# eth-cscs/DLA-Future

Measured on AMD Instinct MI355X. Metric: cholesky_fp64_gflops, higher is better.
Workload: dtype fp64; 1 GPU; model=fp64 Cholesky (POTRF), n=32768, nb=512, parallelism=grid1x1, global_batch=1, seq_len=32768

## Files before the change

csrc/factor.hip:

```cpp
#include <algorithm>

#include "kernels.h"
#include "potrf_plan.h"

namespace {

template <typename S, int BSZ>
__launch_bounds__(256) __global__ void trtri_block_lds_k(const S* L, S* T,
                                                         int n, int ldl,
                                                         int ldt,
                                                         int unit_diag) {
  using TR = ScalarTraits<S>;
  __shared__ S Ts[BSZ][BSZ + 1];
  const int tid = threadIdx.x;
  const int j = tid;
  if (j < n) {
    for (int i = 0; i < j; ++i) Ts[i][j] = TR::zero();
    const S djj = unit_diag ? TR::from_real(1) : TR::recip(L[(int64_t)j * ldl + j]);
    Ts[j][j] = djj;
    for (int i = j + 1; i < n; ++i) {
      S acc = TR::zero();
      const S* Lrow = L + (int64_t)i * ldl;
      for (int p = j; p < i; ++p) acc += Lrow[p] * Ts[p][j];
      const S dii = unit_diag ? TR::from_real(1) : TR::recip(L[(int64_t)i * ldl + i]);
      Ts[i][j] = -(dii * acc);
    }
  }
  __syncthreads();
  for (int e = tid; e < BSZ * BSZ; e += 256) {
    const int i = e / BSZ, j2 = e % BSZ;
    if (i < n && j2 < n) T[(int64_t)i * ldt + j2] = Ts[i][j2];
  }
}

constexpr int kB = dlaf::kPotrfBsz;
constexpr int kImgLd = kB + 1;
static_assert(kB == 64, "the core below is written for 64 x 64 blocks");

template <typename S>
using Img = S (*)[kImgLd];

template <typename S>
__device__ __forceinline__ S read_lane(S v, int src) {
  constexpr int NW = sizeof(S) / 4;
  int w[NW];
  __builtin_memcpy(w, &v, sizeof(S));
#pragma unroll
  for (int q = 0; q < NW; ++q) w[q] = __builtin_amdgcn_readlane(w[q], src);
  __builtin_memcpy(&v, w, sizeof(S));
  return v;
}

__device__ __forceinline__ double pivot_rcp(double a) {
  double x = __builtin_amdgcn_rcp(a);
  double e = fma(-a, x, 1.0);
  x = fma(x, e, x);
  e = fma(-a, x, 1.0);
  return fma(x, e, x);
}
__device__ __forceinline__ float pivot_rcp(float a) { return 1.0f / a; }

template <typename S>
__device__ inline void factor16_wave(Img<S> L,
                                     typename ScalarTraits<S>::real_t* rdiag,
                                     int c0, int lane) {
  using TR = ScalarTraits<S>;
  using RT = typename TR::real_t;
  const int i = lane & 15;
  S u[16];
#pragma unroll
  for (int j = 0; j < 16; ++j) u[j] = L[c0 + i][c0 + j];
#pragma unroll
  for (int p = 0; p < 15; ++p) {
    const RT s = pivot_rcp(TR::real(read_lane(u[p], p)));
    const S w = u[p] * s;
#pragma unroll
    for (int j = p + 1; j < 16; ++j)
      u[j] -= w * TR::conj(read_lane(u[p], j));
  }
  RT dv = RT(0);
#pragma unroll
  for (int j = 0; j < 16; ++j)
    if (i == j) dv = TR::real(u[j]);
  const RT sc = RT(1) / sqrt(dv);
#pragma unroll
  for (int j = 0; j < 16; ++j) u[j] = u[j] * read_lane(sc, j);
  if (lane < 16) {
#pragma unroll
    for (int j = 0; j < 16; ++j)
      if (j <= i) L[c0 + i][c0 + j] = u[j];
    rdiag[c0 + i] = sc;
  }
}

template <typename S>
__device__ inline void invert16_wave(Img<S> L, Img<S> T, int c0, int lane) {
  using TR = ScalarTraits<S>;
  const int i = lane & 15;
  S l[16], t[16];
#pragma unroll
  for (int j = 0; j < 16; ++j) l[j] = L[c0 + i][c0 + j];
  S dv = TR::from_real(1);
#pragma unroll
  for (int j = 0; j < 16; ++j)
    if (i == j) dv = l[j];
  const S rd = TR::recip(dv);
#pragma unroll
  for (int c = 0; c < 16; ++c) t[c] = (c == i) ? rd : TR::zero();
#pragma unroll
  for (int p = 0; p < 15; ++p) {
    const S f = rd * l[p];
#pragma unroll
    for (int c = 0; c <= p; ++c) {
      const S tp = read_lane(t[c], p);
      if (i > p) t[c] -= f * tp;
    }
  }
  if (lane < 16) {
#pragma unroll
    for (int c = 0; c < 16; ++c)
      T[c0 + i][c0 + c] = (c <= i) ? t[c] : TR::zero();
  }
}

template <typename S>
__device__ void factor_invert_core(Img<S> L, Img<S> T, S (*Sc)[33],
                                   typename ScalarTraits<S>::real_t* rdiag,
                                   int tid, int do_factor) {
  using TR = ScalarTraits<S>;
  for (int e = tid; e < kB * kImgLd; e += 256) (&T[0][0])[e] = TR::zero();
  if (do_factor) {
    for (int cb = 0; cb < 4; ++cb) {
      const int c0 = cb * 16;
      if (tid < 64) factor16_wave<S>(L, rdiag, c0, tid);
      __syncthreads();
      if (cb == 3) break;
      {
        const int r = c0 + 16 + tid;
        if (r < kB) {
          S a[16];
#pragma unroll
          for (int p = 0; p < 16; ++p) a[p] = L[r][c0 + p];
#pragma unroll
          for (int j = 0; j < 16; ++j) {
            a[j] = a[j] * rdiag[c0 + j];
#pragma unroll
            for (int q = j + 1; q < 16; ++q)
              a[q] -= a[j] * TR::conj(L[c0 + q][c0 + j]);
          }
#pragma unroll
          for (int p = 0; p < 16; ++p) L[r][c0 + p] = a[p];
        }
        __syncthreads();
      }
      {
        const int t0 = c0 + 16, m = 3 - cb;
        const int ti = tid >> 4, tj = tid & 15;
        for (int bi = 0; bi < m; ++bi) {
          S xi[16];
#pragma unroll
          for (int p = 0; p < 16; ++p) xi[p] = L[t0 + 16 * bi + ti][c0 + p];
          for (int bj = 0; bj <= bi; ++bj) {
            if (bj == bi && tj > ti) continue;
            const int rj = t0 + 16 * bj + tj;
            S acc = TR::zero();
#pragma unroll
            for (int p = 0; p < 16; ++p) acc += xi[p] * TR::conj(L[rj][c0 + p]);
            L[t0 + 16 * bi + ti][rj] -= acc;
          }
        }
        __syncthreads();
      }
    }
  } else {
    __syncthreads();
  }
  invert16_wave<S>(L, T, (tid >> 6) * 16, tid & 63);
  __syncthreads();
  for (int dist = 1; dist < 4; ++dist) {
    const int nblk = 4 - dist;
    for (int e = tid; e < nblk * 256; e += 256) {
      const int b = e >> 8, r = (e & 255) >> 4, c = e & 15;
      const int I = (b + dist) * 16, J = b * 16;
      S acc = TR::zero();
      for (int p = J; p < I; ++p) acc += L[I + r][p] * T[p][J + c];
      Sc[(b >> 1) * 16 + r][(b & 1) * 16 + c] = acc;
    }
    __syncthreads();
    for (int e = tid; e < nblk * 256; e += 256) {
      const int b = e >> 8, r = (e & 255) >> 4, c = e & 15;
      const int I = (b + dist) * 16, J = b * 16;
      S acc = TR::zero();
      for (int p = 0; p <= r; ++p)
        acc += T[I + r][I + p] * Sc[(b >> 1) * 16 + p][(b & 1) * 16 + c];
      T[I + r][J + c] = -acc;
    }
    __syncthreads();
  }
}

template <typename S>
__device__ inline void store_factor_and_inverse(Img<S> L, Img<S> T, S* A,
                                                int n, int ld, S* Tout,
                                                int tid, int store_factor) {
  for (int e = tid; e < kB * kB; e += 256) {
    const int i = e >> 6, j = e & 63;
    if (store_factor && i < n && j <= i) A[(int64_t)i * ld + j] = L[i][j];
    Tout[e] = T[i][j];
  }
}

template <typename S>
__launch_bounds__(256) __global__ void potrf_invert_block_k(S* A, int n,
                                                            int ld, S* Tout,
                                                            int do_factor) {
  using TR = ScalarTraits<S>;
  __shared__ S Li[kB][kImgLd];
  __shared__ S Ti[kB][kImgLd];
  __shared__ S Sc[32][33];
  __shared__ typename TR::real_t Rd[kB];
  const int tid = threadIdx.x;
  for (int e = tid; e < kB * kB; e += 256) {
    const int i = e >> 6, j = e & 63;
    Li[i][j] = (i < n && j <= i) ? A[(int64_t)i * ld + j]
                                 : (i == j ? TR::from_real(1) : TR::zero());
  }
  __syncthreads();
  factor_invert_core<S>(Li, Ti, Sc, Rd, tid, do_factor);
  store_factor_and_inverse<S>(Li, Ti, A, n, ld, Tout, tid, do_factor);
}

template <typename S>
__launch_bounds__(256) __global__ void potrf_step_k(S* A, int n, int ld,
                                                    S* dinv, S* side, int d,
                                                    int nbk) {
  using TR = ScalarTraits<S>;
  namespace plan = dlaf::potrf_plan;
  __shared__ S P0[kB][kImgLd];
  __shared__ S P1[kB][kImgLd];
  __shared__ S Sc[32][33];
  __shared__ typename TR::real_t Rd[kB];
  const int tid = threadIdx.x;
  int I, J;
  plan::block_of((int)blockIdx.x, nbk, d, &I, &J);
  const int c = d - 1;
  const int r0 = I * kB, s0 = J * kB, q0 = c * kB;

  for (int R = d - 1; R < nbk; ++R) {
    if (!plan::copies_row(I, J, nbk, d, R)) continue;
    const S* src = side + plan::side_offset((d - 2) & 1, R, nbk, kB);
    for (int e = tid; e < kB * kB; e += 256) {
      const int i = e >> 6, j = e & 63;
      if (R * kB + i < n)
        A[(int64_t)(R * kB + i) * ld + (q0 - kB) + j] = src[e];
    }
  }

  const S* Dc = dinv + (int64_t)c * kB * kB;
  for (int e = tid; e < kB * kB; e += 256) {
    const int i = e >> 6, j = e & 63;
    P0[i][j] = (r0 + i < n) ? A[(int64_t)(r0 + i) * ld + q0 + j] : TR::zero();
    P1[i][j] = Dc[e];
  }
  __syncthreads();

  const int ty = tid >> 4, tx = tid & 15;
  auto panel_product = [&](S (&x)[4][4]) {
#pragma unroll
    for (int a = 0; a < 4; ++a)
#pragma unroll
      for (int b = 0; b < 4; ++b) x[a][b] = TR::zero();
#pragma unroll
    for (int pb = 0; pb < 4; ++pb) {
      for (int pp = 0; pp < 16; ++pp) {
        const int p = pb * 16 + pp;
        S av[4];
#pragma unroll
        for (int a = 0; a < 4; ++a) av[a] = P0[ty + 16 * a][p];
#pragma unroll
        for (int b = pb; b < 4; ++b) {
          const S dv = TR::conj(P1[tx + 16 * b][p]);
#pragma unroll
          for (int a = 0; a < 4; ++a) x[a][b] += av[a] * dv;
        }
      }
    }
  };

  S xi[4][4], xj[4][4];
  panel_product(xi);
  __syncthreads();
  if (I != J) {
    for (int e = tid; e < kB * kB; e += 256) {
      const int i = e >> 6, j = e & 63;
      P0[i][j] = (s0 + i < n) ? A[(int64_t)(s0 + i) * ld + q0 + j] : TR::zero();
    }
    __syncthreads();
    panel_product(xj);
    __syncthreads();
  }
#pragma unroll
  for (int a = 0; a < 4; ++a)
#pragma unroll
    for (int b = 0; b < 4; ++b) {
      P0[ty + 16 * a][tx + 16 * b] = xi[a][b];
      P1[ty + 16 * a][tx + 16 * b] = (I != J) ? xj[a][b] : xi[a][b];
    }
  if (plan::writes_side(I, J, nbk, d)) {
    S* dst = side + plan::side_offset(c & 1, I, nbk, kB);
#pragma unroll
    for (int a = 0; a < 4; ++a)
#pragma unroll
      for (int b = 0; b < 4; ++b)
        dst[(ty + 16 * a) * kB + tx + 16 * b] = xi[a][b];
  } else if (plan::writes_panel_in_place(I, J, nbk, d)) {
#pragma unroll
    for (int a = 0; a < 4; ++a)
#pragma unroll
      for (int b = 0; b < 4; ++b)
        if (r0 + ty + 16 * a < n)
          A[(int64_t)(r0 + ty + 16 * a) * ld + q0 + tx + 16 * b] = xi[a][b];
  }
  __syncthreads();

  S cv[4][4];
#pragma unroll
  for (int a = 0; a < 4; ++a)
#pragma unroll
    for (int b = 0; b < 4; ++b) {
      const int gr = r0 + ty + 16 * a, gc = s0 + tx + 16 * b;
      const bool live = gr < n && gc < n && (I != J || gc <= gr);
      cv[a][b] = live ? A[(int64_t)gr * ld + gc] : TR::zero();
    }
  for (int q = 0; q < kB; ++q) {
    S av[4], bv[4];
#pragma unroll
    for (int a = 0; a < 4; ++a) av[a] = P0[ty + 16 * a][q];
#pragma unroll
    for (int b = 0; b < 4; ++b) bv[b] = TR::conj(P1[tx + 16 * b][q]);
#pragma unroll
    for (int a = 0; a < 4; ++a)
#pragma unroll
      for (int b = 0; b < 4; ++b) cv[a][b] -= av[a] * bv[b];
  }

  if (!plan::factors(I, J, d)) {
#pragma unroll
    for (int a = 0; a < 4; ++a)
#pragma unroll
      for (int b = 0; b < 4; ++b) {
        const int gr = r0 + ty + 16 * a, gc = s0 + tx + 16 * b;
        if (gr < n && gc < n && (I != J || gc <= gr))
          A[(int64_t)gr * ld + gc] = cv[a][b];
      }
    return;
  }

  __syncthreads();
  const int nl = min(kB, n - r0);
#pragma unroll
  for (int a = 0; a < 4; ++a)
#pragma unroll
    for (int b = 0; b < 4; ++b) {
      const int i = ty + 16 * a, j = tx + 16 * b;
      P0[i][j] = (i < nl && j <= i) ? cv[a][b]
                                    : (i == j ? TR::from_real(1) : TR::zero());
    }
  __syncthreads();
  factor_invert_core<S>(P0, P1, Sc, Rd, tid, 1);
  store_factor_and_inverse<S>(P0, P1, A + (int64_t)r0 * ld + r0, nl, ld,
                              dinv + (int64_t)d * kB * kB, tid, 1);
}

template <typename S>
__global__ void trtri_lower_k(const S* L, S* T, int n, int ldl, int ldt,
                              int unit_diag) {
  using TR = ScalarTraits<S>;
  const int j = blockIdx.x * blockDim.x + threadIdx.x;
  if (j >= n) return;
  for (int i = 0; i < j; ++i) T[(int64_t)i * ldt + j] = TR::zero();
  const S djj = unit_diag ? TR::from_real(1) : TR::recip(L[(int64_t)j * ldl + j]);
  T[(int64_t)j * ldt + j] = djj;
  for (int i = j + 1; i < n; ++i) {
    S acc = TR::zero();
    for (int p = j; p < i; ++p)
      acc += L[(int64_t)i * ldl + p] * T[(int64_t)p * ldt + j];
    const S dii = unit_diag ? TR::from_real(1) : TR::recip(L[(int64_t)i * ldl + i]);
    T[(int64_t)i * ldt + j] = -(dii * acc);
  }
}

}

template <typename S>
void dlaf::potrf_invert_block(S* A, int n, int ld, S* Tout, int do_factor,
                              hipStream_t stream) {
  potrf_invert_block_k<S><<<1, 256, 0, stream>>>(A, n, ld, Tout, do_factor);
}

template <typename S>
void dlaf::potrf_tile_fused(S* A, int n, int ld, S* dinv, S* side,
                            hipStream_t stream) {
  namespace plan = dlaf::potrf_plan;
  if (n <= 0) return;
  const int nbk = plan::nblocks(n, kPotrfBsz);
  potrf_invert_block_k<S>
      <<<1, 256, 0, stream>>>(A, std::min(n, kPotrfBsz), ld, dinv, 1);
  for (int d = 1; d < nbk; ++d)
    potrf_step_k<S>
        <<<plan::grid(nbk, d), 256, 0, stream>>>(A, n, ld, dinv, side, d, nbk);
}

template <typename S>
void dlaf::trtri_lower(const S* L, S* T, int n, int ldl, int ldt,
                       int unit_diag, hipStream_t stream) {
  constexpr int BSZ = sizeof(S) == 16 ? 64 : 128;
  if (n <= BSZ)
    trtri_block_lds_k<S, BSZ>
        <<<1, 256, 0, stream>>>(L, T, n, ldl, ldt, unit_diag);
  else
    trtri_lower_k<S>
        <<<(n + 255) / 256, 256, 0, stream>>>(L, T, n, ldl, ldt, unit_diag);
}

#define INSTANTIATE(S)                                                       \
  template void dlaf::potrf_invert_block(S*, int, int, S*, int, hipStream_t); \
  template void dlaf::potrf_tile_fused(S*, int, int, S*, S*, hipStream_t);    \
  template void dlaf::trtri_lower(const S*, S*, int, int, int, int, hipStream_t);
INSTANTIATE(double)
INSTANTIATE(float)
INSTANTIATE(cplx<double>)
INSTANTIATE(cplx<float>)
#undef INSTANTIATE
```

Baseline: 55190 GFlop/s.

## Use MFMA instructions in potrf step kernel and factor-invert core for real types

```diff
diff --git a/csrc/factor.hip b/csrc/factor.hip
--- a/csrc/factor.hip
+++ b/csrc/factor.hip
@@ -1,6 +1,7 @@
 #include <algorithm>
-
-#include "kernels.h"
+#include <type_traits>
+
+#include "gemm_common.h"
 #include "potrf_plan.h"
 
 namespace {
@@ -41,6 +42,9 @@
 using Img = S (*)[kImgLd];
 
 template <typename S>
+constexpr bool kOnMfma = std::is_same_v<S, double> || std::is_same_v<S, float>;
+
+template <typename S>
 __device__ __forceinline__ S read_lane(S v, int src) {
   constexpr int NW = sizeof(S) / 4;
   int w[NW];
@@ -153,7 +157,28 @@
         }
         __syncthreads();
       }
-      {
+      if constexpr (kOnMfma<S>) {
+        using MF = Mfma<S>;
+        const int t0 = c0 + 16, m = 3 - cb;
+        const int w = tid >> 6, li = tid & 15, lk = (tid & 63) >> 4;
+        for (int e = w; e < m * (m + 1) / 2; e += 4) {
+          const int bi = e >= 3 ? 2 : (e >= 1 ? 1 : 0);
+          const int bj = e - bi * (bi + 1) / 2;
+          const int ri = t0 + 16 * bi, rj = t0 + 16 * bj;
+          typename MF::acc_t c;
+#pragma unroll
+          for (int r = 0; r < 4; ++r) c[r] = L[ri + MF::acc_row(lk, r)][rj + li];
+#pragma unroll
+          for (int k = 0; k < 16; k += 4)
+            c = MF::mma(-L[ri + li][c0 + k + lk], L[rj + li][c0 + k + lk], c);
+#pragma unroll
+          for (int r = 0; r < 4; ++r) {
+            const int row = MF::acc_row(lk, r);
+            if (bj < bi || li <= row) L[ri + row][rj + li] = c[r];
+          }
+        }
+        __syncthreads();
+      } else {
         const int t0 = c0 + 16, m = 3 - cb;
         const int ti = tid >> 4, tj = tid & 15;
         for (int bi = 0; bi < m; ++bi) {
@@ -179,12 +204,26 @@
   __syncthreads();
   for (int dist = 1; dist < 4; ++dist) {
     const int nblk = 4 - dist;
-    for (int e = tid; e < nblk * 256; e += 256) {
-      const int b = e >> 8, r = (e & 255) >> 4, c = e & 15;
-      const int I = (b + dist) * 16, J = b * 16;
-      S acc = TR::zero();
-      for (int p = J; p < I; ++p) acc += L[I + r][p] * T[p][J + c];
-      Sc[(b >> 1) * 16 + r][(b & 1) * 16 + c] = acc;
+    if constexpr (kOnMfma<S>) {
+      using MF = Mfma<S>;
+      const int b = tid >> 6, li = tid & 15, lk = (tid & 63) >> 4;
+      if (b < nblk) {
+        const int I = (b + dist) * 16, J = b * 16;
+        typename MF::acc_t c = {0, 0, 0, 0};
+        for (int p = J; p < I; p += 4)
+          c = MF::mma(L[I + li][p + lk], T[p + lk][J + li], c);
+#pragma unroll
+        for (int r = 0; r < 4; ++r)
+          Sc[(b >> 1) * 16 + MF::acc_row(lk, r)][(b & 1) * 16 + li] = c[r];
+      }
+    } else {
+      for (int e = tid; e < nblk * 256; e += 256) {
+        const int b = e >> 8, r = (e & 255) >> 4, c = e & 15;
+        const int I = (b + dist) * 16, J = b * 16;
+        S acc = TR::zero();
+        for (int p = J; p < I; ++p) acc += L[I + r][p] * T[p][J + c];
+        Sc[(b >> 1) * 16 + r][(b & 1) * 16 + c] = acc;
+      }
     }
     __syncthreads();
     for (int e = tid; e < nblk * 256; e += 256) {
@@ -231,6 +270,236 @@
 }
 
 template <typename S>
+__device__ void step_block_vector(S* A, int n, int ld, S* dinv, S* side, int d,
+                                  int nbk, int I, int J, Img<S> P0, Img<S> P1,
+                                  S (*Sc)[33],
+                                  typename ScalarTraits<S>::real_t* Rd,
+                                  int tid) {
+  using TR = ScalarTraits<S>;
+  namespace plan = dlaf::potrf_plan;
+  const int c = d - 1;
+  const int r0 = I * kB, s0 = J * kB, q0 = c * kB;
+  const int ty = tid >> 4, tx = tid & 15;
+  auto panel_product = [&](S (&x)[4][4]) {
+#pragma unroll
+    for (int a = 0; a < 4; ++a)
+#pragma unroll
+      for (int b = 0; b < 4; ++b) x[a][b] = TR::zero();
+#pragma unroll
+    for (int pb = 0; pb < 4; ++pb) {
+      for (int pp = 0; pp < 16; ++pp) {
+        const int p = pb * 16 + pp;
+        S av[4];
+#pragma unroll
+        for (int a = 0; a < 4; ++a) av[a] = P0[ty + 16 * a][p];
+#pragma unroll
+        for (int b = pb; b < 4; ++b) {
+          const S dv = TR::conj(P1[tx + 16 * b][p]);
+#pragma unroll
+          for (int a = 0; a < 4; ++a) x[a][b] += av[a] * dv;
+        }
+      }
+    }
+  };
+
+  S xi[4][4], xj[4][4];
+  panel_product(xi);
+  __syncthreads();
+  if (I != J) {
+    for (int e = tid; e < kB * kB; e += 256) {
+      const int i = e >> 6, j = e & 63;
+      P0[i][j] = (s0 + i < n) ? A[(int64_t)(s0 + i) * ld + q0 + j] : TR::zero();
+    }
+    __syncthreads();
+    panel_product(xj);
+    __syncthreads();
+  }
+#pragma unroll
+  for (int a = 0; a < 4; ++a)
+#pragma unroll
+    for (int b = 0; b < 4; ++b) {
+      P0[ty + 16 * a][tx + 16 * b] = xi[a][b];
+      P1[ty + 16 * a][tx + 16 * b] = (I != J) ? xj[a][b] : xi[a][b];
+    }
+  if (plan::writes_side(I, J, nbk, d)) {
+    S* dst = side + plan::side_offset(c & 1, I, nbk, kB);
+#pragma unroll
+    for (int a = 0; a < 4; ++a)
+#pragma unroll
+      for (int b = 0; b < 4; ++b)
+        dst[(ty + 16 * a) * kB + tx + 16 * b] = xi[a][b];
+  } else if (plan::writes_panel_in_place(I, J, nbk, d)) {
+#pragma unroll
+    for (int a = 0; a < 4; ++a)
+#pragma unroll
+      for (int b = 0; b < 4; ++b)
+        if (r0 + ty + 16 * a < n)
+          A[(int64_t)(r0 + ty + 16 * a) * ld + q0 + tx + 16 * b] = xi[a][b];
+  }
+  __syncthreads();
+
+  S cv[4][4];
+#pragma unroll
+  for (int a = 0; a < 4; ++a)
+#pragma unroll
+    for (int b = 0; b < 4; ++b) {
+      const int gr = r0 + ty + 16 * a, gc = s0 + tx + 16 * b;
+      const bool live = gr < n && gc < n && (I != J || gc <= gr);
+      cv[a][b] = live ? A[(int64_t)gr * ld + gc] : TR::zero();
+    }
+  for (int q = 0; q < kB; ++q) {
+    S av[4], bv[4];
+#pragma unroll
+    for (int a = 0; a < 4; ++a) av[a] = P0[ty + 16 * a][q];
+#pragma unroll
+    for (int b = 0; b < 4; ++b) bv[b] = TR::conj(P1[tx + 16 * b][q]);
+#pragma unroll
+    for (int a = 0; a < 4; ++a)
+#pragma unroll
+      for (int b = 0; b < 4; ++b) cv[a][b] -= av[a] * bv[b];
+  }
+
+  if (!plan::factors(I, J, d)) {
+#pragma unroll
+    for (int a = 0; a < 4; ++a)
+#pragma unroll
+      for (int b = 0; b < 4; ++b) {
+        const int gr = r0 + ty + 16 * a, gc = s0 + tx + 16 * b;
+        if (gr < n && gc < n && (I != J || gc <= gr))
+          A[(int64_t)gr * ld + gc] = cv[a][b];
+      }
+    return;
+  }
+
+  __syncthreads();
+  const int nl = min(kB, n - r0);
+#pragma unroll
+  for (int a = 0; a < 4; ++a)
+#pragma unroll
+    for (int b = 0; b < 4; ++b) {
+      const int i = ty + 16 * a, j = tx + 16 * b;
+      P0[i][j] = (i < nl && j <= i) ? cv[a][b]
+                                    : (i == j ? TR::from_real(1) : TR::zero());
+    }
+  __syncthreads();
+  factor_invert_core<S>(P0, P1, Sc, Rd, tid, 1);
+  store_factor_and_inverse<S>(P0, P1, A + (int64_t)r0 * ld + r0, nl, ld,
+                              dinv + (int64_t)d * kB * kB, tid, 1);
+}
+
+template <typename S>
+__device__ void step_block_mfma(S* A, int n, int ld, S* dinv, S* side, int d,
+                                int nbk, int I, int J, Img<S> P0, Img<S> P1,
+                                S (*Sc)[33],
+                                typename ScalarTraits<S>::real_t* Rd, int tid) {
+  using MF = Mfma<S>;
+  using acc_t = typename MF::acc_t;
+  namespace plan = dlaf::potrf_plan;
+  const int c = d - 1;
+  const int r0 = I * kB, s0 = J * kB, q0 = c * kB;
+  const int w = tid >> 6, li = tid & 15, lk = (tid & 63) >> 4;
+  const int wr = 16 * w;
+
+  const bool diag = I == J;
+  acc_t cv[4];
+#pragma unroll
+  for (int b = 0; b < 4; ++b)
+#pragma unroll
+    for (int r = 0; r < 4; ++r) {
+      const int gr = r0 + wr + MF::acc_row(lk, r), gc = s0 + 16 * b + li;
+      const bool live = gr < n && gc < n && (!diag || gc <= gr);
+      cv[b][r] = live ? A[(int64_t)gr * ld + gc] : S(0);
+    }
+
+  auto panel_product = [&](acc_t (&x)[4]) {
+#pragma unroll
+    for (int b = 0; b < 4; ++b) x[b] = {0, 0, 0, 0};
+#pragma unroll
+    for (int pb = 0; pb < 4; ++pb)
+#pragma unroll
+      for (int k = 0; k < 16; k += 4) {
+        const int p = pb * 16 + k + lk;
+        const S a = P0[wr + li][p];
+#pragma unroll
+        for (int b = pb; b < 4; ++b)
+          x[b] = MF::mma(a, P1[16 * b + li][p], x[b]);
+      }
+  };
+
+  acc_t xi[4], xj[4];
+  panel_product(xi);
+  __syncthreads();
+  if (I != J) {
+    for (int e = tid; e < kB * kB; e += 256) {
+      const int i = e >> 6, j = e & 63;
+      P0[i][j] = (s0 + i < n) ? A[(int64_t)(s0 + i) * ld + q0 + j] : S(0);
+    }
+    __syncthreads();
+    panel_product(xj);
+    __syncthreads();
+  }
+#pragma unroll
+  for (int b = 0; b < 4; ++b)
+#pragma unroll
+    for (int r = 0; r < 4; ++r) {
+      const int i = wr + MF::acc_row(lk, r), j = 16 * b + li;
+      P0[i][j] = xi[b][r];
+      P1[i][j] = (I != J) ? xj[b][r] : xi[b][r];
+    }
+  if (plan::writes_side(I, J, nbk, d)) {
+    S* dst = side + plan::side_offset(c & 1, I, nbk, kB);
+#pragma unroll
+    for (int b = 0; b < 4; ++b)
+#pragma unroll
+      for (int r = 0; r < 4; ++r)
+        dst[(wr + MF::acc_row(lk, r)) * kB + 16 * b + li] = xi[b][r];
+  } else if (plan::writes_panel_in_place(I, J, nbk, d)) {
+#pragma unroll
+    for (int b = 0; b < 4; ++b)
+#pragma unroll
+      for (int r = 0; r < 4; ++r) {
+        const int gr = r0 + wr + MF::acc_row(lk, r);
+        if (gr < n) A[(int64_t)gr * ld + q0 + 16 * b + li] = xi[b][r];
+      }
+  }
+  __syncthreads();
+
+#pragma unroll 4
+  for (int q = 0; q < kB; q += 4) {
+    const S a = -P0[wr + li][q + lk];
+#pragma unroll
+    for (int b = 0; b < 4; ++b)
+      if (!diag || b <= w) cv[b] = MF::mma(a, P1[16 * b + li][q + lk], cv[b]);
+  }
+
+  if (!plan::factors(I, J, d)) {
+#pragma unroll
+    for (int b = 0; b < 4; ++b)
+#pragma unroll
+      for (int r = 0; r < 4; ++r) {
+        const int gr = r0 + wr + MF::acc_row(lk, r), gc = s0 + 16 * b + li;
+        if (gr < n && gc < n && (!diag || gc <= gr))
+          A[(int64_t)gr * ld + gc] = cv[b][r];
+      }
+    return;
+  }
+
+  __syncthreads();
+  const int nl = min(kB, n - r0);
+#pragma unroll
+  for (int b = 0; b < 4; ++b)
+#pragma unroll
+    for (int r = 0; r < 4; ++r) {
+      const int i = wr + MF::acc_row(lk, r), j = 16 * b + li;
+      P0[i][j] = (i < nl && j <= i) ? cv[b][r] : (i == j ? S(1) : S(0));
+    }
+  __syncthreads();
+  factor_invert_core<S>(P0, P1, Sc, Rd, tid, 1);
+  store_factor_and_inverse<S>(P0, P1, A + (int64_t)r0 * ld + r0, nl, ld,
+                              dinv + (int64_t)d * kB * kB, tid, 1);
+}
+
+template <typename S>
 __launch_bounds__(256) __global__ void potrf_step_k(S* A, int n, int ld,
                                                     S* dinv, S* side, int d,
                                                     int nbk) {
@@ -244,7 +513,7 @@
   int I, J;
   plan::block_of((int)blockIdx.x, nbk, d, &I, &J);
   const int c = d - 1;
-  const int r0 = I * kB, s0 = J * kB, q0 = c * kB;
+  const int r0 = I * kB, q0 = c * kB;
 
   for (int R = d - 1; R < nbk; ++R) {
     if (!plan::copies_row(I, J, nbk, d, R)) continue;
@@ -264,112 +533,11 @@
   }
   __syncthreads();
 
-  const int ty = tid >> 4, tx = tid & 15;
-  auto panel_product = [&](S (&x)[4][4]) {
-#pragma unroll
-    for (int a = 0; a < 4; ++a)
-#pragma unroll
-      for (int b = 0; b < 4; ++b) x[a][b] = TR::zero();
-#pragma unroll
-    for (int pb = 0; pb < 4; ++pb) {
-      for (int pp = 0; pp < 16; ++pp) {
-        const int p = pb * 16 + pp;
-        S av[4];
-#pragma unroll
-        for (int a = 0; a < 4; ++a) av[a] = P0[ty + 16 * a][p];
-#pragma unroll
-        for (int b = pb; b < 4; ++b) {
-          const S dv = TR::conj(P1[tx + 16 * b][p]);
-#pragma unroll
-          for (int a = 0; a < 4; ++a) x[a][b] += av[a] * dv;
-        }
-      }
-    }
-  };
-
-  S xi[4][4], xj[4][4];
-  panel_product(xi);
-  __syncthreads();
-  if (I != J) {
-    for (int e = tid; e < kB * kB; e += 256) {
-      const int i = e >> 6, j = e & 63;
-      P0[i][j] = (s0 + i < n) ? A[(int64_t)(s0 + i) * ld + q0 + j] : TR::zero();
-    }
-    __syncthreads();
-    panel_product(xj);
-    __syncthreads();
-  }
-#pragma unroll
-  for (int a = 0; a < 4; ++a)
-#pragma unroll
-    for (int b = 0; b < 4; ++b) {
-      P0[ty + 16 * a][tx + 16 * b] = xi[a][b];
-      P1[ty + 16 * a][tx + 16 * b] = (I != J) ? xj[a][b] : xi[a][b];
-    }
-  if (plan::writes_side(I, J, nbk, d)) {
-    S* dst = side + plan::side_offset(c & 1, I, nbk, kB);
-#pragma unroll
-    for (int a = 0; a < 4; ++a)
-#pragma unroll
-      for (int b = 0; b < 4; ++b)
-        dst[(ty + 16 * a) * kB + tx + 16 * b] = xi[a][b];
-  } else if (plan::writes_panel_in_place(I, J, nbk, d)) {
-#pragma unroll
-    for (int a = 0; a < 4; ++a)
-#pragma unroll
-      for (int b = 0; b < 4; ++b)
-        if (r0 + ty + 16 * a < n)
-          A[(int64_t)(r0 + ty + 16 * a) * ld + q0 + tx + 16 * b] = xi[a][b];
-  }
-  __syncthreads();
-
-  S cv[4][4];
-#pragma unroll
-  for (int a = 0; a < 4; ++a)
-#pragma unroll
-    for (int b = 0; b < 4; ++b) {
-      const int gr = r0 + ty + 16 * a, gc = s0 + tx + 16 * b;
-      const bool live = gr < n && gc < n && (I != J || gc <= gr);
-      cv[a][b] = live ? A[(int64_t)gr * ld + gc] : TR::zero();
-    }
-  for (int q = 0; q < kB; ++q) {
-    S av[4], bv[4];
-#pragma unroll
-    for (int a = 0; a < 4; ++a) av[a] = P0[ty + 16 * a][q];
-#pragma unroll
-    for (int b = 0; b < 4; ++b) bv[b] = TR::conj(P1[tx + 16 * b][q]);
-#pragma unroll
-    for (int a = 0; a < 4; ++a)
-#pragma unroll
-      for (int b = 0; b < 4; ++b) cv[a][b] -= av[a] * bv[b];
-  }
-
-  if (!plan::factors(I, J, d)) {
-#pragma unroll
-    for (int a = 0; a < 4; ++a)
-#pragma unroll
-      for (int b = 0; b < 4; ++b) {
-        const int gr = r0 + ty + 16 * a, gc = s0 + tx + 16 * b;
-        if (gr < n && gc < n && (I != J || gc <= gr))
-          A[(int64_t)gr * ld + gc] = cv[a][b];
-      }
-    return;
-  }
-
-  __syncthreads();
-  const int nl = min(kB, n - r0);
-#pragma unroll
-  for (int a = 0; a < 4; ++a)
-#pragma unroll
-    for (int b = 0; b < 4; ++b) {
-      const int i = ty + 16 * a, j = tx + 16 * b;
-      P0[i][j] = (i < nl && j <= i) ? cv[a][b]
-                                    : (i == j ? TR::from_real(1) : TR::zero());
-    }
-  __syncthreads();
-  factor_invert_core<S>(P0, P1, Sc, Rd, tid, 1);
-  store_factor_and_inverse<S>(P0, P1, A + (int64_t)r0 * ld + r0, nl, ld,
-                              dinv + (int64_t)d * kB * kB, tid, 1);
+  if constexpr (kOnMfma<S>)
+    step_block_mfma<S>(A, n, ld, dinv, side, d, nbk, I, J, P0, P1, Sc, Rd, tid);
+  else
+    step_block_vector<S>(A, n, ld, dinv, side, d, nbk, I, J, P0, P1, Sc, Rd,
+                         tid);
 }
 
 template <typename S>
```

Measured after the change: 55730 GFlop/s, median of 6. About the same (+1.0%).
